# PecanProject/sipnet

Hardware: NVIDIA B200
Metric: ensemble member-timesteps/sec (higher is better)
Workload: dtype f64

## Files before the change

### sipnet_b200/csrc/sip_comm.cu

```cuda
#include <cuda_runtime.h>
#include <dlfcn.h>
#include <nccl.h>

#include <algorithm>
#include <cmath>
#include <numeric>
#include <cstdio>
#include <cstdlib>
#include <cstring>
#include <string>
#include <vector>

#include "sip_assim.cuh"
#include "sip_gsum.cuh"
#include "sip_handle.h"
#include "sip_jitter.cuh"
#include "sip_resample.cuh"

using namespace sip;

namespace {

struct NcclApi {
  void *lib = nullptr;
  ncclResult_t (*GetUniqueId)(ncclUniqueId *) = nullptr;
  ncclResult_t (*CommInitRank)(ncclComm_t *, int, ncclUniqueId, int) = nullptr;
  ncclResult_t (*CommInitAll)(ncclComm_t *, int, const int *) = nullptr;
  ncclResult_t (*CommDestroy)(ncclComm_t) = nullptr;
  ncclResult_t (*AllReduce)(const void *, void *, size_t, ncclDataType_t, ncclRedOp_t, ncclComm_t, cudaStream_t) = nullptr;
  ncclResult_t (*AllGather)(const void *, void *, size_t, ncclDataType_t, ncclComm_t, cudaStream_t) = nullptr;
  ncclResult_t (*Send)(const void *, size_t, ncclDataType_t, int, ncclComm_t, cudaStream_t) = nullptr;
  ncclResult_t (*Recv)(void *, size_t, ncclDataType_t, int, ncclComm_t, cudaStream_t) = nullptr;
  ncclResult_t (*GroupStart)() = nullptr;
  ncclResult_t (*GroupEnd)() = nullptr;
  const char *(*GetErrorString)(ncclResult_t) = nullptr;
};

const NcclApi *nccl_api() {
  static NcclApi api;
  static bool tried = false;
  if (tried) return api.lib ? &api : nullptr;
  tried = true;
  const char *names[] = {getenv("SIPNET_GPU_NCCL_LIB"), "libnccl.so.2", "libnccl.so"};
  void *lib = nullptr;
  for (const char *n : names) {
    if (!n || !*n) continue;
    lib = dlopen(n, RTLD_NOW | RTLD_GLOBAL);
    if (lib) break;
  }
  if (!lib) return nullptr;
#define SIP_BIND(field, sym)                                              \
  api.field = reinterpret_cast<decltype(api.field)>(dlsym(lib, sym));      \
  if (!api.field) return nullptr;
  SIP_BIND(GetUniqueId, "ncclGetUniqueId")
  SIP_BIND(CommInitRank, "ncclCommInitRank")
  SIP_BIND(CommInitAll, "ncclCommInitAll")
  SIP_BIND(CommDestroy, "ncclCommDestroy")
  SIP_BIND(AllReduce, "ncclAllReduce")
  SIP_BIND(AllGather, "ncclAllGather")
  SIP_BIND(Send, "ncclSend")
  SIP_BIND(Recv, "ncclRecv")
  SIP_BIND(GroupStart, "ncclGroupStart")
  SIP_BIND(GroupEnd, "ncclGroupEnd")
  SIP_BIND(GetErrorString, "ncclGetErrorString")
#undef SIP_BIND
  api.lib = lib;
  return &api;
}

#define CUDA_OK(expr)                                                                              \
  do {                                                                                             \
    cudaError_t e__ = (expr);                                                                      \
    if (e__ != cudaSuccess)                                                                        \
      return fail(SIPNET_GPU_ERR_NO_DEVICE, "%s failed: %s", #expr, cudaGetErrorString(e__));      \
  } while (0)
#define NCCL_OK(expr)                                                                              \
  do {                                                                                             \
    ncclResult_t r__ = (expr);                                                                     \
    if (r__ != ncclSuccess)                                                                        \
      return fail(SIPNET_GPU_ERR_NO_DEVICE, "%s failed: %s", #expr, nccl_api()->GetErrorString(r__)); \
  } while (0)

template <class T>
int grow(T *&p, size_t &cap, size_t need, cudaStream_t stream) {
  if (need <= cap && p) return 0;
  CUDA_OK(cudaStreamSynchronize(stream));
  if (p) cudaFree(p);
  p = nullptr;
  cap = 0;
  CUDA_OK(cudaMalloc((void **)&p, std::max<size_t>(need, 1) * sizeof(T)));
  cap = std::max<size_t>(need, 1);
  return 0;
}

int launched(sipnet_gpu_handle *h, cudaError_t e, const char *what) {
  h->launches++;
  return e == cudaSuccess ? 0 : fail(SIPNET_GPU_ERR_NO_DEVICE, "%s launch failed: %s", what, cudaGetErrorString(e));
}

struct Local {
  sipnet_gpu_handle *h = nullptr;
  ncclComm_t comm = nullptr;
  int rank = 0;
  int64_t rowsCap = 0;
  gs::GsStat *statAll = nullptr;
  double *q2All = nullptr;
  uint32_t *hist = nullptr;
  gs::GsRow *state = nullptr;
  gs::GsTie *tieAll = nullptr;
  uint64_t *emitAll = nullptr;
  int32_t *flags = nullptr;
  unsigned char *xchg = nullptr;
  size_t xchgCap = 0;
};

}

struct sipnet_gpu_comm {
  int nranks = 1;
  bool loopback = false;
  std::vector<Local> local;
  std::vector<int64_t> memberCounts;
  float lastExchangeMs = 0.f, lastSummaryMs = 0.f;
  int lastLevels = 0;
  cudaEvent_t ev0 = nullptr, ev1 = nullptr;
};

namespace {

void free_local(Local &l) {
  if (l.h) cudaSetDevice(l.h->device);
  void *ptrs[] = {l.statAll, l.q2All, l.hist, l.state, l.tieAll, l.emitAll, l.flags, l.xchg};
  for (void *p : ptrs)
    if (p) cudaFree(p);
  l = Local{l.h, l.comm, l.rank};
}

sipnet_gpu_comm team_of_one(sipnet_gpu_handle *h) {
  sipnet_gpu_comm one;
  one.local.resize(1);
  one.local[0].h = h;
  one.memberCounts.assign(1, h->nmembers);
  return one;
}

struct Group {
  const sipnet_gpu_comm *c;
  bool grouped;
  explicit Group(const sipnet_gpu_comm *cc) : c(cc), grouped(cc->nranks > 1 && cc->local.size() > 1) {}
  int begin() const {
    if (grouped) NCCL_OK(nccl_api()->GroupStart());
    return 0;
  }
  int end() const {
    if (grouped) NCCL_OK(nccl_api()->GroupEnd());
    return 0;
  }
};

int sync_all(sipnet_gpu_comm *c) {
  for (Local &l : c->local) {
    CUDA_OK(cudaSetDevice(l.h->device));
    CUDA_OK(cudaStreamSynchronize(l.h->stream));
  }
  return 0;
}

int all_gather_bytes(sipnet_gpu_comm *c, size_t bytesPerRank, void *(*buf)(Local &)) {
  if (c->nranks == 1) return 0;
  if (c->loopback) {
    if (int rc = sync_all(c)) return rc;
    for (Local &to : c->local)
      for (Local &from : c->local)
        if (&to != &from) {
          const size_t off = (size_t)from.rank * bytesPerRank;
          CUDA_OK(cudaMemcpyAsync(static_cast<char *>(buf(to)) + off, static_cast<char *>(buf(from)) + off, bytesPerRank,
                                  cudaMemcpyDeviceToDevice, to.h->stream));
        }
    return sync_all(c);
  }
  const Group g(c);
  if (int rc = g.begin()) return rc;
  for (Local &l : c->local) {
    CUDA_OK(cudaSetDevice(l.h->device));
    char *base = static_cast<char *>(buf(l));
    NCCL_OK(nccl_api()->AllGather(base + (size_t)l.rank * bytesPerRank, base, bytesPerRank, ncclUint8, l.comm, l.h->stream));
  }
  return g.end();
}

int all_reduce_hist(sipnet_gpu_comm *c, size_t words) {
  if (c->nranks == 1) return 0;
  if (c->loopback) {
    if (int rc = sync_all(c)) return rc;
    Local &l0 = c->local[0];
    CUDA_OK(cudaSetDevice(l0.h->device));
    for (size_t i = 1; i < c->local.size(); ++i) CUDA_OK(gs::launch_add_u32(l0.hist, c->local[i].hist, words, l0.h->stream));
    for (size_t i = 1; i < c->local.size(); ++i)
      CUDA_OK(cudaMemcpyAsync(c->local[i].hist, l0.hist, words * sizeof(uint32_t), cudaMemcpyDeviceToDevice, l0.h->stream));
    return sync_all(c);
  }
  const Group g(c);
  if (int rc = g.begin()) return rc;
  for (Local &l : c->local) {
    CUDA_OK(cudaSetDevice(l.h->device));
    NCCL_OK(nccl_api()->AllReduce(l.hist, l.hist, words, ncclUint32, ncclSum, l.comm, l.h->stream));
  }
  return g.end();
}

int ensure_scratch(sipnet_gpu_comm *c, Local &l, int64_t rows) {
  if (rows <= l.rowsCap) return 0;
  const int R = c->nranks;
  sipnet_gpu_handle *h = l.h;
  CUDA_OK(cudaSetDevice(h->device));
  CUDA_OK(cudaStreamSynchronize(h->stream));
  free_local(l);
  CUDA_OK(cudaMalloc((void **)&l.statAll, (size_t)R * rows * sizeof(gs::GsStat)));
  CUDA_OK(cudaMalloc((void **)&l.q2All, (size_t)R * rows * sizeof(double)));
  CUDA_OK(cudaMalloc((void **)&l.hist, (size_t)rows * gs::kGsHistWords * sizeof(uint32_t)));
  CUDA_OK(cudaMalloc((void **)&l.state, (size_t)rows * sizeof(gs::GsRow)));
  CUDA_OK(cudaMalloc((void **)&l.tieAll, (size_t)R * rows * gs::kGsMaxStat * sizeof(gs::GsTie)));
  CUDA_OK(cudaMalloc((void **)&l.emitAll, (size_t)R * rows * gs::kGsMaxStat * gs::kGsEmit * sizeof(uint64_t)));
  CUDA_OK(cudaMalloc((void **)&l.flags, 16));
  l.rowsCap = rows;
  return 0;
}

int team_summaries(sipnet_gpu_comm *c) {
  Local &l0 = c->local[0];
  sipnet_gpu_handle *h0 = l0.h;
  const int64_t n = h0->lastEnd - h0->lastBegin;
  if (n <= 0) return fail(SIPNET_GPU_ERR_BAD_ARGUMENT, "no run range to summarise");
  const int ncols = (int)h0->summaryCols.size();
  if (ncols <= 0 || ncols > gs::kGsMaxCols)
    return fail(SIPNET_GPU_ERR_BAD_ARGUMENT, "cross-rank summaries take 1..%d summary columns", gs::kGsMaxCols);
  if (!h0->mean && !h0->quant) return fail(SIPNET_GPU_ERR_BAD_ARGUMENT, "no summary output was requested at init");
  const int nqTotal = h0->quant ? (int)h0->quantiles.size() : 0;
  const int64_t rows = (int64_t)h0->nsites * ncols * n;
  for (Local &l : c->local) {
    sipnet_gpu_handle *h = l.h;
    if (h->lastEnd - h->lastBegin != n || h->nsites != h0->nsites || (int)h->summaryCols.size() != ncols)
      return fail(SIPNET_GPU_ERR_BAD_ARGUMENT, "the ranks of a team must hold the same sites, columns and run range");
    if (int rc = ensure_scratch(c, l, rows)) return rc;
  }
  std::vector<gs::GsArgs> args(c->local.size());
  for (size_t i = 0; i < c->local.size(); ++i) {
    Local &l = c->local[i];
    sipnet_gpu_handle *h = l.h;
    gs::GsArgs &a = args[i];
    memset(&a, 0, sizeof a);
    a.out = h->out;
    a.ld = h->ld;
    a.nsteps = n;
    a.sites = h->sites;
    a.nsites = (int32_t)h->nsites;
    a.ncols = ncols;
    for (int k = 0; k < ncols; ++k) a.colSlot[k] = h->colSlot[h->summaryCols[(size_t)k]];
    a.nranks = c->nranks;
    a.rank = l.rank;
    a.wantMoments = h->mean != nullptr;
    a.statAll = l.statAll;
    a.q2All = l.q2All;
    a.hist = l.hist;
    a.state = l.state;
    a.tieAll = l.tieAll;
    a.emitAll = l.emitAll;
    a.flags = l.flags;
    a.mean = h->mean;
    a.var = h->var;
    a.quant = h->quant;
    a.nqTotal = nqTotal;
  }
  c->lastLevels = 0;
  std::vector<int> order((size_t)nqTotal);
  std::iota(order.begin(), order.end(), 0);
  std::stable_sort(order.begin(), order.end(), [h0](int i, int j) { return h0->quantiles[(size_t)i] < h0->quantiles[(size_t)j]; });
  for (int q0 = 0; q0 < std::max(nqTotal, 1); q0 += gs::kGsMaxQ) {
    const int nq = std::min(gs::kGsMaxQ, nqTotal - q0);
    for (size_t i = 0; i < c->local.size(); ++i) {
      Local &l = c->local[i];
      gs::GsArgs &a = args[i];
      a.nq = std::max(nq, 0);
      for (int k = 0; k < a.nq; ++k) {
        a.qOut[k] = order[(size_t)(q0 + k)];
        a.probs[k] = l.h->quantiles[(size_t)a.qOut[k]];
      }
      a.wantMoments = (l.h->mean != nullptr && q0 == 0) ? 1 : 0;
      CUDA_OK(cudaSetDevice(l.h->device));
      if (int rc = launched(l.h, gs::launch_pass0(a, l.h->stream), "summary")) return rc;
    }
    if (int rc = all_gather_bytes(c, (size_t)rows * sizeof(gs::GsStat), [](Local &l) -> void * { return l.statAll; })) return rc;
    if (args[0].nq > 0)
      if (int rc = all_reduce_hist(c, (size_t)rows * gs::kGsHistWords)) return rc;
    for (int level = 1; level <= gs::kGsLevels; ++level) {
      for (size_t i = 0; i < c->local.size(); ++i) {
        Local &l = c->local[i];
        CUDA_OK(cudaSetDevice(l.h->device));
        CUDA_OK(cudaMemsetAsync(l.flags, 0, 16, l.h->stream));
        if (int rc = launched(l.h, gs::launch_level(args[i], level, l.h->stream), "summary")) return rc;
      }
      int32_t flag = 0;
      {
        Local &l = c->local[0];
        CUDA_OK(cudaSetDevice(l.h->device));
        CUDA_OK(cudaMemcpyAsync(&flag, l.flags, sizeof flag, cudaMemcpyDeviceToHost, l.h->stream));
        CUDA_OK(cudaStreamSynchronize(l.h->stream));
      }
      if (level == 1 && args[0].wantMoments)
        if (int rc = all_gather_bytes(c, (size_t)rows * sizeof(double), [](Local &l) -> void * { return l.q2All; })) return rc;
      if (!flag) break;
      c->lastLevels = std::max(c->lastLevels, level);
      if (int rc = all_reduce_hist(c, (size_t)rows * gs::kGsHistWords)) return rc;
      if (int rc = all_gather_bytes(c, (size_t)rows * gs::kGsMaxStat * sizeof(gs::GsTie), [](Local &l) -> void * { return l.tieAll; }))
        return rc;
    }
    if (args[0].nq > 0) {
      for (size_t i = 0; i < c->local.size(); ++i) {
        Local &l = c->local[i];
        CUDA_OK(cudaSetDevice(l.h->device));
        if (int rc = launched(l.h, gs::launch_emit(args[i], l.h->stream), "summary")) return rc;
      }
      if (int rc = all_gather_bytes(c, (size_t)rows * gs::kGsMaxStat * gs::kGsEmit * sizeof(uint64_t),
                                    [](Local &l) -> void * { return l.emitAll; }))
        return rc;
    }
    for (size_t i = 0; i < c->local.size(); ++i) {
      Local &l = c->local[i];
      CUDA_OK(cudaSetDevice(l.h->device));
      if (int rc = launched(l.h, gs::launch_finish(args[i], l.h->stream), "summary")) return rc;
    }
  }
  for (Local &l : c->local) l.h->summariesValid = true;
  return 0;
}

}

extern "C" int sipnet_gpu_comm_unique_id(void *id) {
  if (!id) return fail(SIPNET_GPU_ERR_BAD_ARGUMENT, "NULL id");
  const NcclApi *api = nccl_api();
  if (!api) return fail(SIPNET_GPU_ERR_NO_DEVICE, "NCCL (libnccl.so.2) could not be loaded: %s", dlerror());
  ncclUniqueId uid;
  NCCL_OK(api->GetUniqueId(&uid));
  static_assert(sizeof(uid) == SIPNET_GPU_COMM_ID_BYTES, "id size");
  memcpy(id, &uid, sizeof uid);
  return 0;
}

static int finish_comm(sipnet_gpu_comm *c) {
  c->memberCounts.assign((size_t)c->nranks, 0);
  if ((int)c->local.size() == c->nranks) {
    for (const Local &l : c->local) c->memberCounts[(size_t)l.rank] = l.h->nmembers;
    return 0;
  }
  std::vector<int64_t *> dev(c->local.size(), nullptr);
  const Group g(c);
  for (size_t i = 0; i < c->local.size(); ++i) {
    Local &l = c->local[i];
    CUDA_OK(cudaSetDevice(l.h->device));
    CUDA_OK(cudaMalloc((void **)&dev[i], (size_t)c->nranks * sizeof(int64_t)));
    const int64_t mine = l.h->nmembers;
    CUDA_OK(cudaMemcpyAsync(dev[i] + l.rank, &mine, sizeof mine, cudaMemcpyHostToDevice, l.h->stream));
    CUDA_OK(cudaStreamSynchronize(l.h->stream));
  }
  if (int rc = g.begin()) return rc;
  for (size_t i = 0; i < c->local.size(); ++i) {
    Local &l = c->local[i];
    CUDA_OK(cudaSetDevice(l.h->device));
    NCCL_OK(nccl_api()->AllGather(dev[i] + l.rank, dev[i], sizeof(int64_t), ncclUint8, l.comm, l.h->stream));
  }
  if (int rc = g.end()) return rc;
  for (size_t i = 0; i < c->local.size(); ++i) {
    Local &l = c->local[i];
    CUDA_OK(cudaSetDevice(l.h->device));
    CUDA_OK(cudaMemcpyAsync(c->memberCounts.data(), dev[i], (size_t)c->nranks * sizeof(int64_t), cudaMemcpyDeviceToHost,
                            l.h->stream));
    CUDA_OK(cudaStreamSynchronize(l.h->stream));
    cudaFree(dev[i]);
  }
  return 0;
}

extern "C" int sipnet_gpu_comm_init_rank(sipnet_gpu_handle *h, int32_t nranks, int32_t rank, const void *id,
                                         sipnet_gpu_comm **out) {
  if (out) *out = nullptr;
  if (!h || !out) return fail(SIPNET_GPU_ERR_BAD_ARGUMENT, "NULL handle or comm pointer");
  if (nranks < 1 || rank < 0 || rank >= nranks) return fail(SIPNET_GPU_ERR_BAD_ARGUMENT, "bad rank %d of %d", rank, nranks);
  sipnet_gpu_comm *c = new sipnet_gpu_comm();
  c->nranks = nranks;
  c->local.resize(1);
  c->local[0].h = h;
  c->local[0].rank = rank;
  if (nranks > 1) {
    if (!id) {
      delete c;
      return fail(SIPNET_GPU_ERR_BAD_ARGUMENT, "NULL id");
    }
    const NcclApi *api = nccl_api();
    if (!api) {
      delete c;
      return fail(SIPNET_GPU_ERR_NO_DEVICE, "NCCL (libnccl.so.2) could not be loaded: %s", dlerror());
    }
    ncclUniqueId uid;
    memcpy(&uid, id, sizeof uid);
    cudaSetDevice(h->device);
    ncclResult_t r = api->CommInitRank(&c->local[0].comm, nranks, uid, rank);
    if (r != ncclSuccess) {
      delete c;
      return fail(SIPNET_GPU_ERR_NO_DEVICE, "ncclCommInitRank failed: %s", api->GetErrorString(r));
    }
  }
  if (int rc = finish_comm(c)) {
    sipnet_gpu_comm_destroy(c);
    return rc;
  }
  *out = c;
  return 0;
}

extern "C" void sipnet_gpu_comm_destroy(sipnet_gpu_comm *c) {
// ... 1246 lines not shown
```

### sipnet_b200/csrc/sip_gsum.cu

```cuda
#include "sip_gsum.cuh"

#include <algorithm>
#include <type_traits>

namespace sip {
namespace gs {

constexpr int kThreads = 512;
constexpr int kUnroll = 4;
constexpr uint64_t kSent = kGsNoKey;

__host__ __device__ constexpr int bits_after(int level) { return level < 7 ? 11 + 8 * level : 64; }
__host__ __device__ constexpr int shift_of(int level) { return 64 - bits_after(level); }
__host__ __device__ constexpr int bins_of(int level) { return level == 0 ? 2048 : (level < 7 ? 256 : 32); }

__device__ __forceinline__ uint64_t key_of(double x) {
  const uint64_t b = (uint64_t)__double_as_longlong(x);
  return (b & 0x8000000000000000ull) ? ~b : (b | 0x8000000000000000ull);
}
__device__ __forceinline__ double val_of(uint64_t k) {
  const uint64_t b = (k & 0x8000000000000000ull) ? (k & 0x7FFFFFFFFFFFFFFFull) : ~k;
  return __longlong_as_double((long long)b);
}
__device__ __forceinline__ bool finite_hi(double x) { return (((unsigned int)__double2hiint(x) >> 20) & 0x7ffu) != 0x7ffu; }

__device__ __forceinline__ void hist_add(unsigned int *hist, int code) {
  const int lead = __shfl_sync(0xffffffffu, code, 0);
  const unsigned same = __ballot_sync(0xffffffffu, code == lead);
  if ((threadIdx.x & 31) == 0) {
    if (lead >= 0) atomicAdd(&hist[lead], (unsigned)__popc(same));
  } else if (code >= 0 && code != lead) {
    atomicAdd(&hist[code], 1u);
  }
}

__device__ __forceinline__ double block_sum(double v, double *sh) {
  const int tid = threadIdx.x;
  sh[tid] = v;
  __syncthreads();
  for (int s = kThreads / 2; s > 0; s >>= 1) {
    if (tid < s) sh[tid] += sh[tid + s];
    __syncthreads();
  }
  const double r = sh[0];
  __syncthreads();
  return r;
}

struct RowRef {
  const double *p;
  int count;
  int64_t row;
};
__device__ __forceinline__ RowRef row_ref(const GsArgs &a) {
  const int64_t row = blockIdx.x;
  const int64_t t = row % a.nsteps;
  const int64_t sc = row / a.nsteps;
  const int ci = (int)(sc % a.ncols);
  const int site = (int)(sc / a.ncols);
  const SiteDev sd = a.sites[site];
  return RowRef{a.out + ((int64_t)a.colSlot[ci] * a.nsteps + t) * a.ld + sd.member0, sd.memberCount, row};
}

__global__ void __launch_bounds__(kThreads, 2) gs_pass0_kernel(const GsArgs a) {
  __shared__ unsigned int hist[2048];
  __shared__ double red[kThreads];
  __shared__ int repTid;
  __shared__ unsigned long long repKey;
  __shared__ unsigned int diffLo, diffHi;
  const int tid = threadIdx.x;
  const RowRef r = row_ref(a);
  const bool wantHist = a.nq > 0;
  if (wantHist)
    for (int i = tid; i < 2048; i += kThreads) hist[i] = 0;
  if (tid == 0) {
    repTid = kThreads;
    diffLo = diffHi = 0;
  }
  __syncthreads();
  double s = 0.0, c = 0.0;
  uint64_t first = 0, diff = 0;
  bool have = false;
  for (int i0 = 0; i0 < r.count; i0 += kUnroll * kThreads) {
    double x[kUnroll];
#pragma unroll
    for (int u = 0; u < kUnroll; ++u) {
      const int i = i0 + u * kThreads + tid;
      x[u] = i < r.count ? r.p[i] : __longlong_as_double(0x7ff8000000000000ll);
    }
#pragma unroll
    for (int u = 0; u < kUnroll; ++u) {
      const bool fin = finite_hi(x[u]);
      int code = -1;
      if (fin) {
        s += x[u];
        c += 1.0;
        const uint64_t k = key_of(x[u]);
        if (!have) {
          first = k;
          have = true;
        }
        diff |= k ^ first;
        code = (int)(k >> 53);
      }
      if (wantHist) hist_add(hist, code);
    }
  }
  const double total = block_sum(s, red);
  const double n = block_sum(c, red);
  if (have) atomicMin(&repTid, tid);
  __syncthreads();
  if (tid == repTid) repKey = first;
  __syncthreads();
  if (have) {
    diff |= first ^ (uint64_t)repKey;
    if ((unsigned int)diff) atomicOr(&diffLo, (unsigned int)diff);
    if ((unsigned int)(diff >> 32)) atomicOr(&diffHi, (unsigned int)(diff >> 32));
  }
  __syncthreads();
  if (tid == 0) {
    GsStat st;
    st.count = n;
    st.sum = total;
    st.rep = n > 0 ? (uint64_t)repKey : 0;
    st.diff = ((uint64_t)diffHi << 32) | diffLo;
    a.statAll[(int64_t)a.rank * gridDim.x + r.row] = st;
  }
  if (wantHist) {
    unsigned int *g = a.hist + r.row * kGsHistWords;
    for (int i = tid; i < 2048; i += kThreads) g[i] = hist[i];
  }
}

__device__ void init_state(const GsArgs &a, int64_t row, int64_t rows, GsRow &S) {
  double n = 0.0, sum = 0.0;
  bool constant = true, any = false;
  uint64_t rep = 0;
  for (int q = 0; q < a.nranks; ++q) {
    const GsStat st = a.statAll[(int64_t)q * rows + row];
    n += st.count;
    sum += st.sum;
    if (st.count > 0) {
      if (!any) {
        rep = st.rep;
        any = true;
      }
      if (st.diff != 0 || st.rep != rep) constant = false;
    }
  }
  S.n = n;
  S.mean = n > 0 ? sum / n : __longlong_as_double(0x7ff8000000000000ll);
  S.bits = 0;
  S.nslots = 1;
  for (int i = 0; i < kGsMaxStat; ++i) {
    S.prefix[i] = 0;
    S.k[i] = 0;
    S.pop[i] = 0;
    S.slotOf[i] = 0;
    S.rbits[i] = 0;
  }
  if (!(n > 0)) {
    S.done = 3;
  } else if (constant) {
    S.done = 2;
    S.prefix[0] = rep;
  } else {
    S.done = a.nq > 0 ? 0 : 1;
    for (int i = 0; i < a.nq; ++i) {
      const double pos = a.probs[i] * (n - 1.0);
      const double lo = floor(pos);
      const double fr = pos - lo;
      S.k[2 * i] = (uint64_t)lo;
      S.k[2 * i + 1] = (uint64_t)(fr > 0.0 ? lo + 1.0 : lo);
      S.pop[2 * i] = S.pop[2 * i + 1] = 0xffffffffu;
    }
  }
}

__device__ void resolve_level(const GsArgs &a, GsRow &S, const unsigned int *hist, int level) {
  uint8_t *rbits = S.rbits;
  const int warp = threadIdx.x >> 5, lane = threadIdx.x & 31;
  const int nr = 2 * a.nq;
  if (warp < nr && rbits[warp] == 0) {
    const unsigned int *h = level == 0 ? hist : hist + (int)S.slotOf[warp] * 256;
    const int per = bins_of(level) / 32;
    unsigned long long mine = 0;
    for (int b = 0; b < per; ++b) mine += h[lane * per + b];
    unsigned long long incl = mine;
    for (int d = 1; d < 32; d <<= 1) {
      const unsigned long long o = __shfl_up_sync(0xffffffffu, incl, d);
      if (lane >= d) incl += o;
    }
    const unsigned long long k = S.k[warp];
    const unsigned owner = __ballot_sync(0xffffffffu, incl > k);
    const int who = __ffs(owner) - 1;
    __syncwarp();
    if (lane == who) {
      unsigned long long acc = incl - mine;
      int bin = lane * per;
      for (; bin < lane * per + per - 1; ++bin) {
        const unsigned long long cnt = h[bin];
        if (acc + cnt > k) break;
        acc += cnt;
      }
      S.prefix[warp] |= (uint64_t)bin << shift_of(level);
      S.k[warp] = k - acc;
      S.pop[warp] = h[bin];
    }
  }
  __syncthreads();
  if (threadIdx.x == 0) {
    S.bits = (uint8_t)bits_after(level);
    int ns = 0;
    bool done = true;
    for (int r = 0; r < nr; ++r) {
      if (rbits[r] == 0 && (S.pop[r] <= (uint32_t)kGsEmit || S.bits == 64)) rbits[r] = S.bits;
      if (rbits[r] != 0) {
        S.slotOf[r] = 0xff;
        continue;
      }
      done = false;
      int e = 0;
      while (e < r && (rbits[e] != 0 || S.prefix[e] != S.prefix[r])) ++e;
      S.slotOf[r] = e < r ? S.slotOf[e] : (uint8_t)ns++;
    }
    S.nslots = (uint8_t)ns;
    S.done = done ? 1 : 0;
  }
  __syncthreads();
}


template <bool HI32>
__global__ void __launch_bounds__(kThreads, 2) gs_level_kernel(const GsArgs a, const int level) {
  __shared__ unsigned int hist[kGsHistWords];
  __shared__ double red[kThreads];
  __shared__ GsRow S;
  __shared__ uint64_t slotTop[kGsMaxStat];
  __shared__ unsigned long long tieRep[kGsMaxStat];
  __shared__ unsigned int tieLo[kGsMaxStat], tieHi[kGsMaxStat];
  const int tid = threadIdx.x;
  const RowRef r = row_ref(a);
  const int64_t rows = gridDim.x;
  if (level == 1) {
    if (tid == 0) init_state(a, r.row, rows, S);
  } else {
    if (a.state[r.row].done != 0) return;
    if (tid == 0) S = a.state[r.row];
  }
  __syncthreads();
  if (S.done == 0) {
    if (level >= 2 && tid < 2 * a.nq && S.rbits[tid] == 0) {
      const int slot = S.slotOf[tid];
      bool any = false, same = true;
      uint64_t rep = 0;
      for (int q = 0; q < a.nranks; ++q) {
        const GsTie t = a.tieAll[((int64_t)q * rows + r.row) * kGsMaxStat + slot];
        if (t.rep == kGsNoKey) continue;
        if (!any) {
          rep = t.rep;
          any = true;
        }
        if (t.diff != 0 || t.rep != rep) same = false;
      }
      if (any && same) {
        S.prefix[tid] = rep;
        S.rbits[tid] = 64;
      }
    }
    const unsigned int *g = a.hist + r.row * kGsHistWords;
    for (int i = tid; i < kGsHistWords; i += kThreads) hist[i] = g[i];
    __syncthreads();
    resolve_level(a, S, hist, level - 1);
  }
  const bool pass = S.done == 0 && level < kGsLevels;
  const bool needSS = level == 1 && a.wantMoments && S.n > 0;
  if (tid == 0) {
    a.state[r.row] = S;
    if (pass) a.flags[0] = 1;
  }
  if (!pass && !needSS) return;

  const int nslots = S.nslots;
  if (pass) {
    for (int i = tid; i < nslots * 256; i += kThreads) hist[i] = 0;
    if (tid < 2 * a.nq && S.slotOf[tid] != 0xff) slotTop[S.slotOf[tid]] = S.prefix[tid] >> shift_of(level - 1);
    if (tid < kGsMaxStat) {
      tieRep[tid] = kGsNoKey;
      tieLo[tid] = tieHi[tid] = 0;
    }
  }
  __syncthreads();
  const int sh0 = shift_of(level - 1), sh1 = shift_of(level), bmask = bins_of(level) - 1;
  const double mu = S.mean;
  double q2 = 0.0;
  uint64_t top[kGsMaxStat];
  unsigned top32[kGsMaxStat];
#pragma unroll
  for (int s = 0; s < kGsMaxStat; ++s) {
    top[s] = (pass && s < nslots) ? slotTop[s] : kGsNoKey;
    top32[s] = (pass && s < nslots) ? (unsigned)slotTop[s] : 0xffffffffu;
  }
  unsigned trackMask = 0;
  if (pass && level >= 2)
    for (int r2 = 0; r2 < 2 * a.nq; ++r2)
      if (S.slotOf[r2] != 0xff && S.pop[r2] > 1024u) trackMask |= 1u << S.slotOf[r2];
  const auto scan = [&](auto nsTag) {
  constexpr int NS = decltype(nsTag)::value;
  for (int i0 = 0; i0 < r.count; i0 += kUnroll * kThreads) {
    double x[kUnroll];
#pragma unroll
    for (int u = 0; u < kUnroll; ++u) {
      const int i = i0 + u * kThreads + tid;
      x[u] = i < r.count ? r.p[i] : __longlong_as_double(0x7ff8000000000000ll);
    }
#pragma unroll
    for (int u = 0; u < kUnroll; ++u) {
      int code = -1;
      if (finite_hi(x[u])) {
        if (needSS) {
          const double d = x[u] - mu;
          q2 += d * d;
        }
        if (pass) {
          int slot = -1;
          int bin;
          if (HI32) {
            const unsigned hi = (unsigned)__double2hiint(x[u]);
            const unsigned khi = hi ^ ((unsigned)((int)hi >> 31) | 0x80000000u);
            const unsigned t = khi >> (sh0 - 32);
#pragma unroll
            for (int s = 0; s < NS; ++s)
              if (top32[s] == t) slot = s;
            bin = (int)((khi >> (sh1 - 32)) & (unsigned)bmask);
          } else {
            const uint64_t k = key_of(x[u]);
            const uint64_t t = k >> sh0;
#pragma unroll
            for (int s = 0; s < NS; ++s)
              if (top[s] == t) slot = s;
            bin = (int)((k >> sh1) & (uint64_t)bmask);
          }
          if (slot >= 0) {
            code = slot * 256 + bin;
            if ((trackMask >> slot) & 1u) {
              const uint64_t k = key_of(x[u]);
              unsigned long long rep = *(volatile unsigned long long *)&tieRep[slot];
              if (rep == kGsNoKey) {
                const unsigned long long old = atomicCAS(&tieRep[slot], (unsigned long long)kGsNoKey, (unsigned long long)k);
                rep = old == kGsNoKey ? k : old;
              }
              const uint64_t d = k ^ rep;
              if (d) {
                const unsigned int lo = (unsigned int)d, hi2 = (unsigned int)(d >> 32);
                if (lo & ~*(volatile unsigned int *)&tieLo[slot]) atomicOr(&tieLo[slot], lo);
                if (hi2 & ~*(volatile unsigned int *)&tieHi[slot]) atomicOr(&tieHi[slot], hi2);
              }
            }
          }
        }
      }
      if (pass && __any_sync(0xffffffffu, code >= 0)) hist_add(hist, code);
    }
  }
  };
  if (nslots <= 1) scan(std::integral_constant<int, 1>{});
  else if (nslots <= 2) scan(std::integral_constant<int, 2>{});
  else if (nslots <= 4) scan(std::integral_constant<int, 4>{});
  else scan(std::integral_constant<int, kGsMaxStat>{});
  if (needSS) {
    const double ss = block_sum(q2, red);
    if (tid == 0) a.q2All[(int64_t)a.rank * rows + r.row] = ss;
  }
  if (pass) {
    __syncthreads();
    unsigned int *g = a.hist + r.row * kGsHistWords;
    for (int i = tid; i < nslots * 256; i += kThreads) g[i] = hist[i];
    if (tid < kGsMaxStat) {
      GsTie t;
      const bool watched = (trackMask >> tid) & 1u;
      t.rep = watched ? tieRep[tid] : 0;
      t.diff = watched ? (((uint64_t)tieHi[tid] << 32) | tieLo[tid]) : ~0ull;
      a.tieAll[((int64_t)a.rank * rows + r.row) * kGsMaxStat + tid] = t;
    }
  }
}

__global__ void __launch_bounds__(kThreads, 2) gs_emit_kernel(const GsArgs a) {
  __shared__ GsRow S;
  __shared__ uint64_t top[kGsMaxStat];
  __shared__ int sh[kGsMaxStat];
  __shared__ int owner[kGsMaxStat];
  __shared__ unsigned int fill[kGsMaxStat];
  __shared__ int nemit;
  const int tid = threadIdx.x;
  const RowRef r = row_ref(a);
  const int64_t rows = gridDim.x;
  const GsRow *gx = a.state + r.row;
  uint64_t *dst = a.emitAll + ((int64_t)a.rank * rows + r.row) * (kGsMaxStat * kGsEmit);
  for (int i = tid; i < kGsMaxStat * kGsEmit; i += kThreads) dst[i] = kSent;
  if (gx->done != 1 || a.nq == 0) return;
  if (tid == 0) {
    S = *gx;
    int ne = 0;
    for (int s = 0; s < 2 * a.nq; ++s) {
      fill[s] = 0;
      owner[s] = -1;
      if (S.rbits[s] >= 64) continue;
      const int shv = 64 - (int)S.rbits[s];
      bool shared = false;
      for (int e = 0; e < s; ++e)
        if (owner[e] == e && S.rbits[e] == S.rbits[s] && (S.prefix[e] >> shv) == (S.prefix[s] >> shv)) {
          owner[s] = e;
          shared = true;
          break;
        }
      if (!shared) {
        owner[s] = s;
        ++ne;
      }
      top[s] = S.prefix[s] >> shv;
      sh[s] = shv;
    }
    nemit = ne;
  }
  __syncthreads();
  if (nemit == 0) return;
  uint64_t tp[kGsMaxStat];
  unsigned tp32[kGsMaxStat];
  int shv[kGsMaxStat], at[kGsMaxStat];
  bool hi32 = true;
  {
    int j = 0;
#pragma unroll
    for (int s = 0; s < kGsMaxStat; ++s) {
      tp[s] = kGsNoKey;
      tp32[s] = 0xffffffffu;
      shv[s] = 32;
      at[s] = 0;
    }
#pragma unroll
    for (int s = 0; s < kGsMaxStat; ++s) {
      const bool on = s < 2 * a.nq && owner[s] == s;
      if (on) {
#pragma unroll
        for (int jj = 0; jj < kGsMaxStat; ++jj)
          if (jj == j) {
            tp[jj] = top[s];
            tp32[jj] = (unsigned)top[s];
            shv[jj] = sh[s];
            at[jj] = s;
          }
        if (sh[s] < 32) hi32 = false;
        ++j;
      }
    }
  }
  const auto scan = [&](auto neTag) {
    constexpr int NE = decltype(neTag)::value;
    for (int i0 = 0; i0 < r.count; i0 += kUnroll * kThreads) {
      double x[kUnroll];
#pragma unroll
      for (int u = 0; u < kUnroll; ++u) {
        const int i = i0 + u * kThreads + tid;
        x[u] = i < r.count ? r.p[i] : __longlong_as_double(0x7ff8000000000000ll);
      }
#pragma unroll
      for (int u = 0; u < kUnroll; ++u) {
        if (!finite_hi(x[u])) continue;
        if (hi32) {
          const unsigned hi = (unsigned)__double2hiint(x[u]);
          const unsigned khi = hi ^ ((unsigned)((int)hi >> 31) | 0x80000000u);
          int hit = -1;
#pragma unroll
          for (int j = 0; j < NE; ++j)
            if ((khi >> (shv[j] - 32)) == tp32[j]) hit = at[j];
          if (hit >= 0) {
            const unsigned int pos = atomicAdd(&fill[hit], 1u);
            if (pos < (unsigned)kGsEmit) dst[hit * kGsEmit + pos] = key_of(x[u]);
          }
        } else {
          const uint64_t k = key_of(x[u]);
#pragma unroll
          for (int j = 0; j < NE; ++j) {
            if ((k >> shv[j]) == tp[j]) {
              const unsigned int pos = atomicAdd(&fill[at[j]], 1u);
              if (pos < (unsigned)kGsEmit) dst[at[j] * kGsEmit + pos] = k;
            }
          }
        }
      }
    }
  };
  if (nemit <= 1) scan(std::integral_constant<int, 1>{});
  else if (nemit <= 2) scan(std::integral_constant<int, 2>{});
  else if (nemit <= 4) scan(std::integral_constant<int, 4>{});
  else scan(std::integral_constant<int, kGsMaxStat>{});
}

__global__ void gs_finish_kernel(const GsArgs a, const int64_t rows) {
  const int64_t row = (int64_t)blockIdx.x * (blockDim.x / 32) + (threadIdx.x >> 5);
  const int lane = threadIdx.x & 31;
  if (row >= rows) return;
  const GsRow *gx = a.state + row;
  const int64_t t = row % a.nsteps;
  const int64_t sc = row / a.nsteps;
  const double nanv = __longlong_as_double(0x7ff8000000000000ll);
  const int done = gx->done;
  const int nr = 2 * a.nq;
  uint64_t key = 0;
  if (done == 1 && lane < nr) {
    const int s = lane;
    const int rb = gx->rbits[s];
    if (rb >= 64) {
      key = gx->prefix[s];
    } else {
      const int shv = 64 - rb;
      int e = s;
      for (int j = 0; j < s; ++j)
        if (gx->rbits[j] == rb && (gx->prefix[j] >> shv) == (gx->prefix[s] >> shv)) {
          e = j;
          break;
        }
      uint64_t c[kGsEmit];
      int nc = 0;
      for (int q = 0; q < a.nranks; ++q) {
        const uint64_t *src = a.emitAll + (((int64_t)q * rows + row) * kGsMaxStat + e) * kGsEmit;
        for (int i = 0; i < kGsEmit && nc < kGsEmit; ++i) {
          const uint64_t v = src[i];
          if (v == kSent) break;
          int p = nc++;
          while (p > 0 && c[p - 1] > v) {
            c[p] = c[p - 1];
            --p;
          }
          c[p] = v;
        }
      }
      const uint64_t kk = gx->k[s];
      key = kk < (uint64_t)nc ? c[kk] : kSent;
    }
  }
  for (int i = 0; i < a.nq; ++i) {
    const uint64_t klo = __shfl_sync(0xffffffffu, key, 2 * i);
    const uint64_t khi = __shfl_sync(0xffffffffu, key, 2 * i + 1);
    if (lane != i) continue;
    double v = nanv;
    if (done == 2) {
      v = val_of(gx->prefix[0]);
    } else if (done == 1) {
      const double n = gx->n;
      const double pos = a.probs[i] * (n - 1.0);
      const double fr = pos - floor(pos);
      const double xlo = val_of(klo), xhi = val_of(khi);
      v = (fr >= 0.5) ? xhi - (xhi - xlo) * (1.0 - fr) : xlo + (xhi - xlo) * fr;
    }
    a.quant[(sc * a.nqTotal + a.qOut[i]) * a.nsteps + t] = v;
  }
  if (a.wantMoments && lane == 0) {
    const double n = gx->n;
    double ss = 0.0;
    if (n > 0)
      for (int q = 0; q < a.nranks; ++q) ss += a.q2All[(int64_t)q * rows + row];
    a.mean[sc * a.nsteps + t] = gx->mean;
    a.var[sc * a.nsteps + t] = n > 0 ? ss / n : nanv;
  }
}

cudaError_t launch_pass0(const GsArgs &a, cudaStream_t stream) {
  gs_pass0_kernel<<<(unsigned)gs_rows(a), kThreads, 0, stream>>>(a);
  return cudaGetLastError();
}
cudaError_t launch_level(const GsArgs &a, int level, cudaStream_t stream) {
  if (level <= 2) gs_level_kernel<true><<<(unsigned)gs_rows(a), kThreads, 0, stream>>>(a, level);
  else gs_level_kernel<false><<<(unsigned)gs_rows(a), kThreads, 0, stream>>>(a, level);
  return cudaGetLastError();
}
cudaError_t launch_emit(const GsArgs &a, cudaStream_t stream) {
  gs_emit_kernel<<<(unsigned)gs_rows(a), kThreads, 0, stream>>>(a);
  return cudaGetLastError();
}
cudaError_t launch_finish(const GsArgs &a, cudaStream_t stream) {
  const int64_t rows = gs_rows(a);
  gs_finish_kernel<<<(unsigned)((rows + 3) / 4), 128, 0, stream>>>(a, rows);
  return cudaGetLastError();
}

__global__ void add_u32_kernel(uint32_t *dst, const uint32_t *src, size_t n) {
  for (size_t i = (size_t)blockIdx.x * blockDim.x + threadIdx.x; i < n; i += (size_t)gridDim.x * blockDim.x) dst[i] += src[i];
}
cudaError_t launch_add_u32(uint32_t *dst, const uint32_t *src, size_t n, cudaStream_t stream) {
  const size_t blocks = std::min<size_t>((n + 255) / 256, 4096);
  add_u32_kernel<<<(unsigned)std::max<size_t>(blocks, 1), 256, 0, stream>>>(dst, src, n);
  return cudaGetLastError();
}

}
}
```

### sipnet_b200/csrc/sip_gsum.cuh

```cuda
#pragma once
#include <cuda_runtime.h>

#include <cstdint>

#include "sip_types.cuh"

namespace sip {
namespace gs {

constexpr int kGsMaxQ = 4;
constexpr int kGsMaxStat = 2 * kGsMaxQ;
constexpr int kGsEmit = 16;
constexpr int kGsHistWords = 2048;
constexpr int kGsLevels = 8;
constexpr int kGsMaxCols = 8;

struct GsStat {
  double count, sum;
  uint64_t rep;
  uint64_t diff;
};

struct GsTie {
  uint64_t rep;
  uint64_t diff;
};
constexpr uint64_t kGsNoKey = ~0ull;

struct GsRow {
  uint64_t prefix[kGsMaxStat];
  uint64_t k[kGsMaxStat];
  uint32_t pop[kGsMaxStat];
  uint8_t slotOf[kGsMaxStat];
  uint8_t rbits[kGsMaxStat];
  uint8_t nslots;
  uint8_t bits;
  uint8_t done;
  uint8_t pad;
  double n, mean;
};

struct GsArgs {
  const double *out;
  int64_t ld, nsteps;
  const SiteDev *sites;
  int32_t nsites, ncols;
  int32_t colSlot[kGsMaxCols];
  int32_t nq;
  double probs[kGsMaxQ];
  int32_t qOut[kGsMaxQ];
  int32_t nranks, rank;
  int32_t wantMoments;
  GsStat *statAll;
  double *q2All;
  uint32_t *hist;
  GsRow *state;
  GsTie *tieAll;
  uint64_t *emitAll;
  int32_t *flags;
  double *mean, *var, *quant;
  int32_t nqTotal;
};

inline int64_t gs_rows(const GsArgs &a) { return (int64_t)a.nsites * a.ncols * a.nsteps; }

cudaError_t launch_pass0(const GsArgs &a, cudaStream_t stream);
cudaError_t launch_level(const GsArgs &a, int level, cudaStream_t stream);
cudaError_t launch_emit(const GsArgs &a, cudaStream_t stream);
cudaError_t launch_finish(const GsArgs &a, cudaStream_t stream);
cudaError_t launch_add_u32(uint32_t *dst, const uint32_t *src, size_t n, cudaStream_t stream);

}
}
```

Before: 10.43 billion.

## Collect small candidate sets during radix-select passes to resolve quantiles early

During the multi-level radix select used for ensemble quantile summaries, each row block now writes the raw keys of small candidate buckets into a per-row buffer while it scans. Later levels pick the exact order statistic by sorting these kept candidates instead of running further histogram passes. This applies only to single-rank runs and is meant to cut the number of full data scans per row. The cost is extra global writes, atomics and shared memory in the scan loop, plus a new scratch allocation.

```diff
diff --git a/sipnet_b200/csrc/sip_comm.cu b/sipnet_b200/csrc/sip_comm.cu
--- a/sipnet_b200/csrc/sip_comm.cu
+++ b/sipnet_b200/csrc/sip_comm.cu
@@ -109,6 +109,8 @@
   gs::GsRow *state = nullptr;
   gs::GsTie *tieAll = nullptr;
   uint64_t *emitAll = nullptr;
+  uint64_t *kept = nullptr;
+  uint32_t *keptInfo = nullptr;
   int32_t *flags = nullptr;
   unsigned char *xchg = nullptr;
   size_t xchgCap = 0;
@@ -130,7 +132,7 @@
 
 void free_local(Local &l) {
   if (l.h) cudaSetDevice(l.h->device);
-  void *ptrs[] = {l.statAll, l.q2All, l.hist, l.state, l.tieAll, l.emitAll, l.flags, l.xchg};
+  void *ptrs[] = {l.statAll, l.q2All, l.hist, l.state, l.tieAll, l.emitAll, l.kept, l.keptInfo, l.flags, l.xchg};
   for (void *p : ptrs)
     if (p) cudaFree(p);
   l = Local{l.h, l.comm, l.rank};
@@ -222,6 +224,10 @@
   CUDA_OK(cudaMalloc((void **)&l.state, (size_t)rows * sizeof(gs::GsRow)));
   CUDA_OK(cudaMalloc((void **)&l.tieAll, (size_t)R * rows * gs::kGsMaxStat * sizeof(gs::GsTie)));
   CUDA_OK(cudaMalloc((void **)&l.emitAll, (size_t)R * rows * gs::kGsMaxStat * gs::kGsEmit * sizeof(uint64_t)));
+  if (R == 1) {
+    CUDA_OK(cudaMalloc((void **)&l.kept, (size_t)rows * gs::kGsCollect * sizeof(uint64_t)));
+    CUDA_OK(cudaMalloc((void **)&l.keptInfo, (size_t)rows * 2 * sizeof(uint32_t)));
+  }
   CUDA_OK(cudaMalloc((void **)&l.flags, 16));
   l.rowsCap = rows;
   return 0;
@@ -266,6 +272,8 @@
     a.state = l.state;
     a.tieAll = l.tieAll;
     a.emitAll = l.emitAll;
+    a.kept = l.kept;
+    a.keptInfo = l.keptInfo;
     a.flags = l.flags;
     a.mean = h->mean;
     a.var = h->var;
diff --git a/sipnet_b200/csrc/sip_gsum.cu b/sipnet_b200/csrc/sip_gsum.cu
--- a/sipnet_b200/csrc/sip_gsum.cu
+++ b/sipnet_b200/csrc/sip_gsum.cu
@@ -231,7 +231,43 @@
 }
 
 
-template <bool HI32>
+__device__ void take_kept(const GsArgs &a, GsRow &S, const uint8_t *slot0, int64_t row) {
+  __shared__ uint64_t sel[kGsMaxStat][kGsEmit];
+  __shared__ unsigned int nsel[kGsMaxStat];
+  const int tid = threadIdx.x, nr = 2 * a.nq;
+  const unsigned mask = a.keptInfo[2 * row], n = min(a.keptInfo[2 * row + 1], (unsigned)kGsCollect);
+  if (mask == 0) return;
+  const auto taken = [&](int q) { return slot0[q] != 0xff && ((mask >> slot0[q]) & 1u) && S.rbits[q] != 0 && S.rbits[q] < 64; };
+  if (tid < kGsMaxStat) nsel[tid] = 0;
+  __syncthreads();
+  const uint64_t *kept = a.kept + row * kGsCollect;
+  for (unsigned i = tid; i < n; i += kThreads) {
+    const uint64_t c = kept[i];
+    for (int q = 0; q < nr; ++q) {
+      if (!taken(q)) continue;
+      const int shv = 64 - S.rbits[q];
+      if ((c >> shv) != (S.prefix[q] >> shv)) continue;
+      const unsigned p = atomicAdd(&nsel[q], 1u);
+      if (p < (unsigned)kGsEmit) sel[q][p] = c;
+    }
+  }
+  __syncthreads();
+  if (tid < nr && taken(tid)) {
+    uint64_t *c = sel[tid];
+    const int nc = (int)min(nsel[tid], (unsigned)kGsEmit);
+    for (int i = 1; i < nc; ++i) {
+      const uint64_t v = c[i];
+      int p = i;
+      for (; p > 0 && c[p - 1] > v; --p) c[p] = c[p - 1];
+      c[p] = v;
+    }
+    S.prefix[tid] = S.k[tid] < (uint64_t)nc ? c[S.k[tid]] : kSent;
+    S.rbits[tid] = 64;
+  }
+  __syncthreads();
+}
+
+template <bool HI32, bool KEEP>
 __global__ void __launch_bounds__(kThreads, 2) gs_level_kernel(const GsArgs a, const int level) {
   __shared__ unsigned int hist[kGsHistWords];
   __shared__ double red[kThreads];
@@ -239,6 +275,8 @@
   __shared__ uint64_t slotTop[kGsMaxStat];
   __shared__ unsigned long long tieRep[kGsMaxStat];
   __shared__ unsigned int tieLo[kGsMaxStat], tieHi[kGsMaxStat];
+  __shared__ uint8_t slot0[kGsMaxStat];
+  __shared__ unsigned int ncand, collectMask;
   const int tid = threadIdx.x;
   const RowRef r = row_ref(a);
   const int64_t rows = gridDim.x;
@@ -270,8 +308,10 @@
     }
     const unsigned int *g = a.hist + r.row * kGsHistWords;
     for (int i = tid; i < kGsHistWords; i += kThreads) hist[i] = g[i];
+    if (tid < kGsMaxStat) slot0[tid] = (tid < 2 * a.nq && S.rbits[tid] == 0) ? S.slotOf[tid] : 0xff;
     __syncthreads();
     resolve_level(a, S, hist, level - 1);
+    if (a.kept && level >= 3) take_kept(a, S, slot0, r.row);
   }
   const bool pass = S.done == 0 && level < kGsLevels;
   const bool needSS = level == 1 && a.wantMoments && S.n > 0;
@@ -289,6 +329,18 @@
       tieRep[tid] = kGsNoKey;
       tieLo[tid] = tieHi[tid] = 0;
     }
+    if (tid == 0) {
+      unsigned m = 0, left = kGsCollect;
+      if (KEEP && a.kept)
+        for (int r2 = 0; r2 < 2 * a.nq; ++r2) {
+          const int sl = S.slotOf[r2];
+          if (sl == 0xff || ((m >> sl) & 1u) || S.pop[r2] > left) continue;
+          m |= 1u << sl;
+          left -= S.pop[r2];
+        }
+      collectMask = m;
+      ncand = 0;
+    }
   }
   __syncthreads();
   const int sh0 = shift_of(level - 1), sh1 = shift_of(level), bmask = bins_of(level) - 1;
@@ -305,6 +357,7 @@
   if (pass && level >= 2)
     for (int r2 = 0; r2 < 2 * a.nq; ++r2)
       if (S.slotOf[r2] != 0xff && S.pop[r2] > 1024u) trackMask |= 1u << S.slotOf[r2];
+  const unsigned keepMask = (KEEP && pass) ? collectMask : 0u;
   const auto scan = [&](auto nsTag) {
   constexpr int NS = decltype(nsTag)::value;
   for (int i0 = 0; i0 < r.count; i0 += kUnroll * kThreads) {
@@ -360,7 +413,21 @@
           }
         }
       }
-      if (pass && __any_sync(0xffffffffu, code >= 0)) hist_add(hist, code);
+      if (pass && __any_sync(0xffffffffu, code >= 0)) {
+        hist_add(hist, code);
+        if (KEEP && keepMask) {
+          const bool keep = code >= 0 && ((keepMask >> (code >> 8)) & 1u);
+          const unsigned m = __ballot_sync(0xffffffffu, keep);
+          if (m) {
+            const int lane = tid & 31, lead = __ffs(m) - 1;
+            unsigned base = 0;
+            if (lane == lead) base = atomicAdd(&ncand, (unsigned)__popc(m));
+            base = __shfl_sync(0xffffffffu, base, lead);
+            const unsigned pos = base + (unsigned)__popc(m & ((1u << lane) - 1u));
+            if (keep && pos < (unsigned)kGsCollect) a.kept[r.row * kGsCollect + pos] = key_of(x[u]);
+          }
+        }
+      }
     }
   }
   };
@@ -383,6 +450,10 @@
       t.diff = watched ? (((uint64_t)tieHi[tid] << 32) | tieLo[tid]) : ~0ull;
       a.tieAll[((int64_t)a.rank * rows + r.row) * kGsMaxStat + tid] = t;
     }
+  }
+  if (KEEP && pass && a.kept && tid == 0) {
+    a.keptInfo[2 * r.row] = keepMask;
+    a.keptInfo[2 * r.row + 1] = ncand;
   }
 }
 
@@ -572,8 +643,9 @@
   return cudaGetLastError();
 }
 cudaError_t launch_level(const GsArgs &a, int level, cudaStream_t stream) {
-  if (level <= 2) gs_level_kernel<true><<<(unsigned)gs_rows(a), kThreads, 0, stream>>>(a, level);
-  else gs_level_kernel<false><<<(unsigned)gs_rows(a), kThreads, 0, stream>>>(a, level);
+  if (level == 1) gs_level_kernel<true, false><<<(unsigned)gs_rows(a), kThreads, 0, stream>>>(a, level);
+  else if (level == 2) gs_level_kernel<true, true><<<(unsigned)gs_rows(a), kThreads, 0, stream>>>(a, level);
+  else gs_level_kernel<false, true><<<(unsigned)gs_rows(a), kThreads, 0, stream>>>(a, level);
   return cudaGetLastError();
 }
 cudaError_t launch_emit(const GsArgs &a, cudaStream_t stream) {
diff --git a/sipnet_b200/csrc/sip_gsum.cuh b/sipnet_b200/csrc/sip_gsum.cuh
--- a/sipnet_b200/csrc/sip_gsum.cuh
+++ b/sipnet_b200/csrc/sip_gsum.cuh
@@ -11,6 +11,7 @@
 constexpr int kGsMaxQ = 4;
 constexpr int kGsMaxStat = 2 * kGsMaxQ;
 constexpr int kGsEmit = 16;
+constexpr int kGsCollect = 2048;
 constexpr int kGsHistWords = 2048;
 constexpr int kGsLevels = 8;
 constexpr int kGsMaxCols = 8;
@@ -57,6 +58,8 @@
   GsRow *state;
   GsTie *tieAll;
   uint64_t *emitAll;
+  uint64_t *kept;
+  uint32_t *keptInfo;
   int32_t *flags;
   double *mean, *var, *quant;
   int32_t nqTotal;
```

Measured after the change: 10.59 billion, median of 6. 1.6% higher.

## Compact surviving candidates into per-row lists for later radix-select levels

Applied to the files above, without the earlier changes.

Once the total population of the quantile candidate buckets in a row falls below a cap, the level kernel writes those candidate values into a per-row compact list. Later levels and the emit pass then scan only that list instead of rereading the full ensemble column. The pass-0 and high-32-bit scans also use a wider unroll, and the warp histogram add is made branchless. This adds scratch memory plus extra atomics and shared-memory bookkeeping on the level where the list is filled.

```diff
diff --git a/sipnet_b200/csrc/sip_comm.cu b/sipnet_b200/csrc/sip_comm.cu
--- a/sipnet_b200/csrc/sip_comm.cu
+++ b/sipnet_b200/csrc/sip_comm.cu
@@ -110,6 +110,8 @@
   gs::GsTie *tieAll = nullptr;
   uint64_t *emitAll = nullptr;
   int32_t *flags = nullptr;
+  double *list = nullptr;
+  int32_t *listN = nullptr;
   unsigned char *xchg = nullptr;
   size_t xchgCap = 0;
 };
@@ -130,7 +132,7 @@
 
 void free_local(Local &l) {
   if (l.h) cudaSetDevice(l.h->device);
-  void *ptrs[] = {l.statAll, l.q2All, l.hist, l.state, l.tieAll, l.emitAll, l.flags, l.xchg};
+  void *ptrs[] = {l.statAll, l.q2All, l.hist, l.state, l.tieAll, l.emitAll, l.flags, l.list, l.listN, l.xchg};
   for (void *p : ptrs)
     if (p) cudaFree(p);
   l = Local{l.h, l.comm, l.rank};
@@ -209,8 +211,8 @@
   return g.end();
 }
 
-int ensure_scratch(sipnet_gpu_comm *c, Local &l, int64_t rows) {
-  if (rows <= l.rowsCap) return 0;
+int ensure_scratch(sipnet_gpu_comm *c, Local &l, int64_t rows, bool lists) {
+  if (rows <= l.rowsCap && (!lists || l.list)) return 0;
   const int R = c->nranks;
   sipnet_gpu_handle *h = l.h;
   CUDA_OK(cudaSetDevice(h->device));
@@ -223,6 +225,10 @@
   CUDA_OK(cudaMalloc((void **)&l.tieAll, (size_t)R * rows * gs::kGsMaxStat * sizeof(gs::GsTie)));
   CUDA_OK(cudaMalloc((void **)&l.emitAll, (size_t)R * rows * gs::kGsMaxStat * gs::kGsEmit * sizeof(uint64_t)));
   CUDA_OK(cudaMalloc((void **)&l.flags, 16));
+  if (lists) {
+    CUDA_OK(cudaMalloc((void **)&l.list, (size_t)rows * gs::kGsListCap * sizeof(double)));
+    CUDA_OK(cudaMalloc((void **)&l.listN, (size_t)rows * sizeof(int32_t)));
+  }
   l.rowsCap = rows;
   return 0;
 }
@@ -242,7 +248,8 @@
     sipnet_gpu_handle *h = l.h;
     if (h->lastEnd - h->lastBegin != n || h->nsites != h0->nsites || (int)h->summaryCols.size() != ncols)
       return fail(SIPNET_GPU_ERR_BAD_ARGUMENT, "the ranks of a team must hold the same sites, columns and run range");
-    if (int rc = ensure_scratch(c, l, rows)) return rc;
+    const bool lists = nqTotal > 0 && h->ld >= 4 * (int64_t)gs::kGsListCap * h->nsites;
+    if (int rc = ensure_scratch(c, l, rows, lists)) return rc;
   }
   std::vector<gs::GsArgs> args(c->local.size());
   for (size_t i = 0; i < c->local.size(); ++i) {
@@ -267,6 +274,8 @@
     a.tieAll = l.tieAll;
     a.emitAll = l.emitAll;
     a.flags = l.flags;
+    a.list = l.list;
+    a.listN = l.listN;
     a.mean = h->mean;
     a.var = h->var;
     a.quant = h->quant;
diff --git a/sipnet_b200/csrc/sip_gsum.cu b/sipnet_b200/csrc/sip_gsum.cu
--- a/sipnet_b200/csrc/sip_gsum.cu
+++ b/sipnet_b200/csrc/sip_gsum.cu
@@ -8,6 +8,7 @@
 
 constexpr int kThreads = 512;
 constexpr int kUnroll = 4;
+constexpr int kUnrollWide = 8;
 constexpr uint64_t kSent = kGsNoKey;
 
 __host__ __device__ constexpr int bits_after(int level) { return level < 7 ? 11 + 8 * level : 64; }
@@ -27,11 +28,8 @@
 __device__ __forceinline__ void hist_add(unsigned int *hist, int code) {
   const int lead = __shfl_sync(0xffffffffu, code, 0);
   const unsigned same = __ballot_sync(0xffffffffu, code == lead);
-  if ((threadIdx.x & 31) == 0) {
-    if (lead >= 0) atomicAdd(&hist[lead], (unsigned)__popc(same));
-  } else if (code >= 0 && code != lead) {
-    atomicAdd(&hist[code], 1u);
-  }
+  const bool first = (threadIdx.x & 31) == 0;
+  if (code >= 0 && (first || code != lead)) atomicAdd(&hist[code], first ? (unsigned)__popc(same) : 1u);
 }
 
 __device__ __forceinline__ double block_sum(double v, double *sh) {
@@ -81,15 +79,15 @@
   double s = 0.0, c = 0.0;
   uint64_t first = 0, diff = 0;
   bool have = false;
-  for (int i0 = 0; i0 < r.count; i0 += kUnroll * kThreads) {
-    double x[kUnroll];
-#pragma unroll
-    for (int u = 0; u < kUnroll; ++u) {
+  for (int i0 = 0; i0 < r.count; i0 += kUnrollWide * kThreads) {
+    double x[kUnrollWide];
+#pragma unroll
+    for (int u = 0; u < kUnrollWide; ++u) {
       const int i = i0 + u * kThreads + tid;
       x[u] = i < r.count ? r.p[i] : __longlong_as_double(0x7ff8000000000000ll);
     }
 #pragma unroll
-    for (int u = 0; u < kUnroll; ++u) {
+    for (int u = 0; u < kUnrollWide; ++u) {
       const bool fin = finite_hi(x[u]);
       int code = -1;
       if (fin) {
@@ -152,6 +150,7 @@
   S.mean = n > 0 ? sum / n : __longlong_as_double(0x7ff8000000000000ll);
   S.bits = 0;
   S.nslots = 1;
+  S.listed = 0;
   for (int i = 0; i < kGsMaxStat; ++i) {
     S.prefix[i] = 0;
     S.k[i] = 0;
@@ -239,6 +238,9 @@
   __shared__ uint64_t slotTop[kGsMaxStat];
   __shared__ unsigned long long tieRep[kGsMaxStat];
   __shared__ unsigned int tieLo[kGsMaxStat], tieHi[kGsMaxStat];
+  __shared__ uint64_t xTop[kGsMaxStat];
+  __shared__ int xSh[kGsMaxStat], nx;
+  __shared__ unsigned int listFill;
   const int tid = threadIdx.x;
   const RowRef r = row_ref(a);
   const int64_t rows = gridDim.x;
@@ -276,12 +278,39 @@
   const bool pass = S.done == 0 && level < kGsLevels;
   const bool needSS = level == 1 && a.wantMoments && S.n > 0;
   if (tid == 0) {
+    nx = 0;
+    listFill = 0;
+    if (pass && a.list && S.listed == 0) {
+      uint64_t popSum = 0;
+      for (int q = 0; q < 2 * a.nq; ++q) {
+        bool first = true;
+        if (S.rbits[q] == 0) {
+          for (int e = 0; e < q; ++e) first = first && !(S.rbits[e] == 0 && S.slotOf[e] == S.slotOf[q]);
+          if (first) popSum += S.pop[q];
+        } else if (S.rbits[q] < 64) {
+          const int shv = 64 - (int)S.rbits[q];
+          for (int e = 0; e < nx; ++e) first = first && !(xSh[e] == shv && xTop[e] == S.prefix[q] >> shv);
+          if (first) {
+            popSum += S.pop[q];
+            xTop[nx] = S.prefix[q] >> shv;
+            xSh[nx++] = shv;
+          }
+        }
+      }
+      if (popSum <= (uint64_t)kGsListCap) S.listed = (uint8_t)level;
+    }
     a.state[r.row] = S;
     if (pass) a.flags[0] = 1;
   }
+  __syncthreads();
   if (!pass && !needSS) return;
 
   const int nslots = S.nslots;
+  const bool fromList = S.listed != 0 && S.listed < level;
+  const bool listing = pass && S.listed == level;
+  const double *src = fromList ? a.list + r.row * kGsListCap : r.p;
+  const int count = fromList ? a.listN[r.row] : r.count;
+  double *dstList = a.list + r.row * kGsListCap;
   if (pass) {
     for (int i = tid; i < nslots * 256; i += kThreads) hist[i] = 0;
     if (tid < 2 * a.nq && S.slotOf[tid] != 0xff) slotTop[S.slotOf[tid]] = S.prefix[tid] >> shift_of(level - 1);
@@ -305,18 +334,22 @@
   if (pass && level >= 2)
     for (int r2 = 0; r2 < 2 * a.nq; ++r2)
       if (S.slotOf[r2] != 0xff && S.pop[r2] > 1024u) trackMask |= 1u << S.slotOf[r2];
-  const auto scan = [&](auto nsTag) {
+  const int nxs = nx;
+  const auto scan = [&](auto nsTag, auto listTag) {
   constexpr int NS = decltype(nsTag)::value;
-  for (int i0 = 0; i0 < r.count; i0 += kUnroll * kThreads) {
-    double x[kUnroll];
-#pragma unroll
-    for (int u = 0; u < kUnroll; ++u) {
+  constexpr bool LIST = decltype(listTag)::value;
+  constexpr int UN = HI32 ? kUnrollWide : kUnroll;
+  for (int i0 = 0; i0 < count; i0 += UN * kThreads) {
+    double x[UN];
+#pragma unroll
+    for (int u = 0; u < UN; ++u) {
       const int i = i0 + u * kThreads + tid;
-      x[u] = i < r.count ? r.p[i] : __longlong_as_double(0x7ff8000000000000ll);
-    }
-#pragma unroll
-    for (int u = 0; u < kUnroll; ++u) {
+      x[u] = i < count ? src[i] : __longlong_as_double(0x7ff8000000000000ll);
+    }
+#pragma unroll
+    for (int u = 0; u < UN; ++u) {
       int code = -1;
+      bool keep = false;
       if (finite_hi(x[u])) {
         if (needSS) {
           const double d = x[u] - mu;
@@ -340,6 +373,13 @@
             for (int s = 0; s < NS; ++s)
               if (top[s] == t) slot = s;
             bin = (int)((k >> sh1) & (uint64_t)bmask);
+          }
+          if (LIST) {
+            keep = slot >= 0;
+            if (nxs > 0) {
+              const uint64_t k = key_of(x[u]);
+              for (int j = 0; j < nxs; ++j) keep = keep || (k >> xSh[j]) == xTop[j];
+            }
           }
           if (slot >= 0) {
             code = slot * 256 + bin;
@@ -360,20 +400,37 @@
           }
         }
       }
-      if (pass && __any_sync(0xffffffffu, code >= 0)) hist_add(hist, code);
+      if (!LIST) {
+        if (pass && __any_sync(0xffffffffu, code >= 0)) hist_add(hist, code);
+      } else {
+        const unsigned m = __ballot_sync(0xffffffffu, keep);
+        if (m) {
+          hist_add(hist, code);
+          const int lane = tid & 31;
+          unsigned base = 0;
+          if (lane == 0) base = atomicAdd(&listFill, (unsigned)__popc(m));
+          base = __shfl_sync(0xffffffffu, base, 0) + (unsigned)__popc(m & ((1u << lane) - 1u));
+          if (keep && base < (unsigned)kGsListCap) dstList[base] = x[u];
+        }
+      }
     }
   }
   };
-  if (nslots <= 1) scan(std::integral_constant<int, 1>{});
-  else if (nslots <= 2) scan(std::integral_constant<int, 2>{});
-  else if (nslots <= 4) scan(std::integral_constant<int, 4>{});
-  else scan(std::integral_constant<int, kGsMaxStat>{});
+  const auto slots = [&](auto listTag) {
+    if (nslots <= 1) scan(std::integral_constant<int, 1>{}, listTag);
+    else if (nslots <= 2) scan(std::integral_constant<int, 2>{}, listTag);
+    else if (nslots <= 4) scan(std::integral_constant<int, 4>{}, listTag);
+    else scan(std::integral_constant<int, kGsMaxStat>{}, listTag);
+  };
+  if (listing) slots(std::true_type{});
+  else slots(std::false_type{});
   if (needSS) {
     const double ss = block_sum(q2, red);
     if (tid == 0) a.q2All[(int64_t)a.rank * rows + r.row] = ss;
   }
   if (pass) {
     __syncthreads();
+    if (listing && tid == 0) a.listN[r.row] = (int)min(listFill, (unsigned)kGsListCap);
     unsigned int *g = a.hist + r.row * kGsHistWords;
     for (int i = tid; i < nslots * 256; i += kThreads) g[i] = hist[i];
     if (tid < kGsMaxStat) {
@@ -426,6 +483,9 @@
   }
   __syncthreads();
   if (nemit == 0) return;
+  const bool fromList = S.listed != 0;
+  const double *src = fromList ? a.list + r.row * kGsListCap : r.p;
+  const int count = fromList ? a.listN[r.row] : r.count;
   uint64_t tp[kGsMaxStat];
   unsigned tp32[kGsMaxStat];
   int shv[kGsMaxStat], at[kGsMaxStat];
@@ -458,12 +518,12 @@
   }
   const auto scan = [&](auto neTag) {
     constexpr int NE = decltype(neTag)::value;
-    for (int i0 = 0; i0 < r.count; i0 += kUnroll * kThreads) {
+    for (int i0 = 0; i0 < count; i0 += kUnroll * kThreads) {
       double x[kUnroll];
 #pragma unroll
       for (int u = 0; u < kUnroll; ++u) {
         const int i = i0 + u * kThreads + tid;
-        x[u] = i < r.count ? r.p[i] : __longlong_as_double(0x7ff8000000000000ll);
+        x[u] = i < count ? src[i] : __longlong_as_double(0x7ff8000000000000ll);
       }
 #pragma unroll
       for (int u = 0; u < kUnroll; ++u) {
diff --git a/sipnet_b200/csrc/sip_gsum.cuh b/sipnet_b200/csrc/sip_gsum.cuh
--- a/sipnet_b200/csrc/sip_gsum.cuh
+++ b/sipnet_b200/csrc/sip_gsum.cuh
@@ -14,6 +14,7 @@
 constexpr int kGsHistWords = 2048;
 constexpr int kGsLevels = 8;
 constexpr int kGsMaxCols = 8;
+constexpr int kGsListCap = 4096;
 
 struct GsStat {
   double count, sum;
@@ -36,7 +37,7 @@
   uint8_t nslots;
   uint8_t bits;
   uint8_t done;
-  uint8_t pad;
+  uint8_t listed;
   double n, mean;
 };
 
@@ -58,6 +59,8 @@
   GsTie *tieAll;
   uint64_t *emitAll;
   int32_t *flags;
+  double *list;
+  int32_t *listN;
   double *mean, *var, *quant;
   int32_t nqTotal;
 };
```

Result: faster. 10.44 billion before, 10.75 billion after (median of 6 runs) (+3.0%).
